# isl-org/Open3D-PointNet2-Semantic3D

Hardware: AMD Instinct MI355X
Metric: points/sec through SA+FP stack (B=16,N=8192) (higher is better)
Workload: dtype f32

## Files before the change

### open3d-pointnet2-semantic3d_amd/csrc/pn2_common.h

```cpp
#pragma once
#include <hip/hip_runtime.h>
#include <stdint.h>

#include "../../include/pn2_abi.h"
#include "pn2_device_set.h"

#define PN2_WAVE 64

#ifdef PN2_TUNING_HOOKS
#define PN2_TUNABLE(type, name, value) type name = value;
#else
#define PN2_TUNABLE(type, name, value) static constexpr type name = value;
#endif

#define PN2_RETURN_IF_LAUNCH_FAILED()                 \
    do {                                              \
        hipError_t e__ = hipGetLastError();           \
        if (e__ != hipSuccess) return (int)e__;       \
    } while (0)

constexpr int kPn2CuLdsBytes = 160 * 1024;
constexpr int kPn2DefaultDynLdsBytes = 64 * 1024;

template <auto Kern>
int pn2_allow_lds(int bytes) {
    static Pn2DeviceSet raised;
    int dev = -1;
    hipError_t e = hipGetDevice(&dev);
    if (e != hipSuccess) return (int)e;
    if (raised.done(dev)) return 0;
    e = hipFuncSetAttribute(reinterpret_cast<const void*>(Kern), hipFuncAttributeMaxDynamicSharedMemorySize, bytes);
    if (e != hipSuccess) return (int)e;
    raised.mark(dev);
    return 0;
}

constexpr int kPn2BnHead = 48;
constexpr int kPn2BnSlots = 64;
constexpr int kPn2BnTickets = 64;
#ifndef PN2_STREAM_MIN_ROWS
#define PN2_STREAM_MIN_ROWS 65536
#endif
#ifndef PN2_FOLD_DEPTH
#define PN2_FOLD_DEPTH 64
#endif
constexpr int kPn2FoldDepth = PN2_FOLD_DEPTH;
__host__ __device__ inline size_t pn2_bn_ws_doubles(int c, int nslots) { return kPn2BnHead + (size_t)(1 + nslots) * 2 * (size_t)c; }
inline bool pn2_bn_ws_fits(const void* ws, size_t bytes, int c) {
    return c > 0 && bytes >= sizeof(double) * pn2_bn_ws_doubles(c, kPn2BnSlots) && ((uintptr_t)ws % 8) == 0;
}

__device__ __forceinline__ void bn_scale_shift(float gamma, float beta, float mean, float invstd, float& sc, float& sh) {
    sc = gamma * invstd;
    sh = __builtin_fmaf(-mean, sc, beta);
}

struct Pn2BnFinish {
    int kind;
    int c, nslots;
    long long rows;
    double* ws;
    const float* gamma;
    const float* beta;
    const float* bias;
    const float* mean_in;
    const float* invstd_in;
    float eps, decay;
    float* running_mean;
    float* running_var;
    float* save_mean;
    float* save_invstd;
    float* scale;
    float* shift;
    float* coef;
    float* dgamma;
    float* dbeta;
};

__device__ __forceinline__ double pn2_load_device_scope(const double* p) {
    return __longlong_as_double((long long)__hip_atomic_load(reinterpret_cast<const unsigned long long*>(p), __ATOMIC_RELAXED,
                                                             __HIP_MEMORY_SCOPE_AGENT));
}

__device__ __forceinline__ void pn2_bn_finish(const Pn2BnFinish& f, unsigned nwg, unsigned wg) {
    if (f.kind == 0) return;
    __shared__ int s_last;
    asm volatile("s_waitcnt vmcnt(0)" ::: "memory");
    __syncthreads();
    if (threadIdx.x == 0) {
        unsigned* tick = reinterpret_cast<unsigned*>(f.ws);
        const unsigned g = wg % (unsigned)kPn2BnTickets;
        const unsigned ng = nwg < (unsigned)kPn2BnTickets ? nwg : (unsigned)kPn2BnTickets;
        const unsigned expect = nwg / kPn2BnTickets + (g < nwg % kPn2BnTickets ? 1u : 0u);
        int last = 0;
        if (__hip_atomic_fetch_add(tick + g, 1u, __ATOMIC_RELAXED, __HIP_MEMORY_SCOPE_AGENT) == expect - 1u)
            last = __hip_atomic_fetch_add(tick + kPn2BnTickets, 1u, __ATOMIC_RELAXED, __HIP_MEMORY_SCOPE_AGENT) == ng - 1u;
        s_last = last;
    }
    __syncthreads();
    if (!s_last) return;
    const int c = f.c;
    for (int col = threadIdx.x; col < 2 * c; col += blockDim.x) {
        double t = 0.0;
        const double* sl = f.ws + kPn2BnHead + (size_t)2 * c + col;
        int k = 0;
        for (; k + kPn2FoldDepth <= f.nslots; k += kPn2FoldDepth) {
            double v[kPn2FoldDepth];
#pragma unroll
            for (int u = 0; u < kPn2FoldDepth; ++u) v[u] = pn2_load_device_scope(sl + (size_t)2 * c * (k + u));
#pragma unroll
            for (int u = 0; u < kPn2FoldDepth; ++u) t += v[u];
        }
        for (; k < f.nslots; ++k) t += pn2_load_device_scope(sl + (size_t)2 * c * k);
        f.ws[kPn2BnHead + col] = t;
    }
    if (f.kind == 1) return;
    __threadfence_block();
    __syncthreads();
// ... 148 lines not shown
```

### open3d-pointnet2-semantic3d_amd/csrc/pn2_mlp_wide.hip

```cpp
#include "pn2_common.h"

namespace {

typedef float f32x4 __attribute__((ext_vector_type(4)));
typedef float f32x16 __attribute__((ext_vector_type(16)));

constexpr int kWideDepth = 4;

struct WideParams {
    int rows, cin, x_stride, nlayers, pool, relu_last;
    int w[3];
    const float* x;
    int n, m, c;
    const float* xyz;
    const float* new_xyz;
    const float* points;
    const int* idx;
    const float* dist;
    const float* points1;
    int c1, c2;
    const float* W[3];
    const float* bias[3];
    float* y;
    const float* zpre;
    int rowtab_off;
    int sa[2];
    int scratch_off;
    int scratch_alias;
};

enum { kWidePlain = 0, kWideGather = 1, kWideInterp = 2 };
template <int MODE>
__global__ void __launch_bounds__(256, 2)
mlp_wide_kernel(WideParams p) {
    constexpr bool GATHER = MODE == kWideGather;
    extern __shared__ __attribute__((aligned(16))) float smem[];
    const int tid = threadIdx.x;
    const int lane = tid & 63, half = lane >> 5, l31 = lane & 31;
    const int wave = __builtin_amdgcn_readfirstlane(tid >> 6);
    const int tile = blockIdx.x;
    const int row0 = tile * 32;
    const int buf_off[2] = {0, 32 * p.sa[0]};
    float* const buf0 = smem;

    struct LayerCfg { int N, wnt, ks_n, nq, ks, cb, g0, g1; const float* wcol; };
    auto make_cfg = [&](int l, int Kt) {
        LayerCfg c;
        c.N = p.w[l];
        c.wnt = c.N >> 7;
        c.ks_n = 4 / c.wnt;
        c.nq = wave % c.wnt;
        c.ks = wave / c.wnt;
        c.cb = c.nq * 128;
        const int ngroups = (Kt + 7) >> 3;
        c.g0 = (ngroups * c.ks) / c.ks_n;
        c.g1 = (ngroups * (c.ks + 1)) / c.ks_n;
        c.wcol = p.W[l] + c.cb + 4 * l31;
        return c;
    };
    f32x4 bq[kWideDepth][4];
    auto fetch_b = [&](const LayerCfg& c, int g, f32x4 (&b_)[4]) {
        const float* __restrict__ wp = c.wcol + (size_t)(8 * g + 4 * half) * c.N;
#pragma unroll
        for (int q = 0; q < 4; ++q) b_[q] = *reinterpret_cast<const f32x4*>(wp + (size_t)q * c.N);
    };
    auto prefetch_b = [&](const LayerCfg& c) {
#pragma unroll
        for (int u = 0; u < kWideDepth; ++u) fetch_b(c, c.g0 + u < c.g1 ? c.g0 + u : c.g1 - 1, bq[u]);
    };
    const LayerCfg first = make_cfg(0, p.cin);
    prefetch_b(first);

    const int K0 = (p.cin + 7) & ~7;
    auto stage4 = [&](int count4, int cv, int sa, auto src_of) {
        for (int base = 0; base < count4; base += 256 * 8) {
            f32x4 v[8];
#pragma unroll
            for (int u = 0; u < 8; ++u) {
                int e = base + u * 256 + tid;
                e = e < count4 ? e : count4 - 1;
                const int r = e / cv, j = e - r * cv;
                v[u] = *reinterpret_cast<const f32x4*>(src_of(r, j));
            }
#pragma unroll
            for (int u = 0; u < 8; ++u) {
                const int e = base + u * 256 + tid;
                if (e < count4) {
                    const int r = e / cv, j = e - r * cv;
                    *reinterpret_cast<f32x4*>(buf0 + r * sa + 4 * j) = v[u];
                }
            }
        }
    };
    if constexpr (GATHER) {
        const int c = p.c, cv = c >> 2;
        const int bi = tile / p.m;
        const float* __restrict__ pts = p.points + (size_t)bi * p.n * c;
        const int* __restrict__ idx = p.idx + (size_t)tile * 32;
        float* myrow = buf0 + (tid & 31) * p.sa[0];
        float dx = 0.f, dy = 0.f, dz = 0.f;
        if (tid < 32) {
            const float* __restrict__ q = p.xyz + ((size_t)bi * p.n + idx[tid]) * 3;
            const float* __restrict__ ctr = p.new_xyz + (size_t)tile * 3;
            dx = q[0] - ctr[0]; dy = q[1] - ctr[1]; dz = q[2] - ctr[2];
        }
        if (p.zpre) {
            if (tid < 32) {
                myrow[0] = dx; myrow[1] = dy; myrow[2] = dz;
                for (int k = 3; k < K0; ++k) myrow[k] = 0.f;
            }
        } else {
        stage4(32 * cv, cv, p.sa[0], [&](int r, int j) { return pts + (size_t)idx[r] * c + 4 * j; });
        if (tid < 32) {
            myrow[c] = dx; myrow[c + 1] = dy; myrow[c + 2] = dz;
            for (int k = c + 3; k < K0; ++k) myrow[k] = 0.f;
        }
        }
    } else if constexpr (MODE == kWideInterp) {
        const int c2 = p.c2, c1 = p.c1, cv2 = c2 >> 2, cv1 = c1 >> 2;
        const int bi = row0 / p.n;
        const float* __restrict__ p2 = p.points + (size_t)bi * p.m * c2;
        float* rowtab = smem + (p.zpre ? p.rowtab_off : buf_off[1]);
        if (tid < 32) {
            const size_t r = (size_t)row0 + tid;
            const float d1 = fmaxf(p.dist[r * 3 + 0], 1e-10f), d2 = fmaxf(p.dist[r * 3 + 1], 1e-10f);
            const float d3 = fmaxf(p.dist[r * 3 + 2], 1e-10f);
            const float r1 = 1.0f / d1, r2 = 1.0f / d2, r3 = 1.0f / d3;
            const float norm = (r1 + r2) + r3;
            *reinterpret_cast<f32x4*>(rowtab + tid * 8) = f32x4{r1 / norm, r2 / norm, r3 / norm, 0.f};
            *reinterpret_cast<f32x4*>(rowtab + tid * 8 + 4) =
                f32x4{__int_as_float(p.idx[r * 3 + 0]), __int_as_float(p.idx[r * 3 + 1]), __int_as_float(p.idx[r * 3 + 2]), 0.f};
        }
        __syncthreads();
        const int count4 = p.zpre ? 0 : 32 * cv2;
        for (int base = 0; base < count4; base += 256 * 4) {
            f32x4 v[4];
#pragma unroll
            for (int u = 0; u < 4; ++u) {
                int e = base + u * 256 + tid;
                e = e < count4 ? e : count4 - 1;
                const int r = e / cv2, j = e - r * cv2;
                const f32x4 wq = *reinterpret_cast<const f32x4*>(rowtab + r * 8);
                const f32x4 iq = *reinterpret_cast<const f32x4*>(rowtab + r * 8 + 4);
                const f32x4 x1 = *reinterpret_cast<const f32x4*>(p2 + (size_t)__float_as_int(iq[0]) * c2 + 4 * j);
                const f32x4 x2 = *reinterpret_cast<const f32x4*>(p2 + (size_t)__float_as_int(iq[1]) * c2 + 4 * j);
                const f32x4 x3 = *reinterpret_cast<const f32x4*>(p2 + (size_t)__float_as_int(iq[2]) * c2 + 4 * j);
                v[u] = (x1 * wq[0] + x2 * wq[1]) + x3 * wq[2];
            }
#pragma unroll
            for (int u = 0; u < 4; ++u) {
                const int e = base + u * 256 + tid;
                if (e < count4) {
                    const int r = e / cv2, j = e - r * cv2;
                    *reinterpret_cast<f32x4*>(buf0 + r * p.sa[0] + 4 * j) = v[u];
                }
            }
        }
        if (c1 > 0) {
            const float* __restrict__ p1 = p.points1 + (size_t)row0 * c1;
            for (int e = tid; e < 32 * cv1; e += 256) {
                const int r = e / cv1, j = e - r * cv1;
                *reinterpret_cast<f32x4*>(buf0 + r * p.sa[0] + (p.zpre ? 0 : c2) + 4 * j) = *reinterpret_cast<const f32x4*>(p1 + (size_t)r * c1 + 4 * j);
            }
        }
        if (K0 > p.cin) {
            const int padw = K0 - p.cin;
            for (int e = tid; e < 32 * padw; e += 256) buf0[(e / padw) * p.sa[0] + p.cin + e % padw] = 0.f;
        }
    } else {
        const float* __restrict__ x = p.x;
        if ((p.x_stride & 3) == 0 && (p.cin & 3) == 0 && (((uintptr_t)x) & 15) == 0) {
            const int cv = p.cin >> 2;
            stage4(32 * cv, cv, p.sa[0], [&](int r, int j) {
                const int gr = row0 + r < p.rows ? row0 + r : p.rows - 1;
                return x + (size_t)gr * p.x_stride + 4 * j;
            });
            if (row0 + 32 > p.rows) {
                __syncthreads();
                for (int e = tid; e < 32 * p.cin; e += 256) {
                    const int r = e / p.cin;
                    if (row0 + r >= p.rows) buf0[r * p.sa[0] + e - r * p.cin] = 0.f;
                }
            }
        } else {
// ... 50 lines not shown
            f32x4 aq[kWideDepth];
#pragma unroll
            for (int u = 0; u < kWideDepth; ++u) aq[u] = *reinterpret_cast<const f32x4*>(arow + 8 * (g0 + u < g1 ? g0 + u : last));
            int g = g0;
            for (; g + 2 * kWideDepth <= g1; g += kWideDepth) {
#pragma unroll
                for (int u = 0; u < kWideDepth; ++u) {
                    contract(aq[u], bq[u]);
                    __builtin_amdgcn_sched_barrier(0);
                    const int gn = g + kWideDepth + u;
                    aq[u] = *reinterpret_cast<const f32x4*>(arow + 8 * gn);
                    fetch_b(cur, gn, bq[u]);
                    __builtin_amdgcn_sched_barrier(0);
                }
            }
            const int rem = g1 - g - kWideDepth;
#pragma unroll
            for (int u = 0; u < kWideDepth; ++u) {
                if (g + u < g1) contract(aq[u], bq[u]);
                if (u < rem) {
                    aq[u] = *reinterpret_cast<const f32x4*>(arow + 8 * (g + kWideDepth + u));
                    fetch_b(cur, g + kWideDepth + u, bq[u]);
                }
            }
#pragma unroll
            for (int u = 0; u < kWideDepth - 1; ++u)
                if (u < rem) contract(aq[u], bq[u]);
        }
        const bool lastl = l == p.nlayers - 1;
        LayerCfg nxt = cur;
        if (!lastl) {
            nxt = make_cfg(l + 1, N);
            prefetch_b(nxt);
        }

        if (ks_n > 1) {
            const int sc_off = p.scratch_alias ? in_off : p.scratch_off;
            if (p.scratch_alias) __syncthreads();
            auto park = [&](int block) {
                float* dst = smem + sc_off + block * (64 * 64);
#pragma unroll
                for (int t = 0; t < 4; ++t)
#pragma unroll
                    for (int r = 0; r < 16; ++r) dst[(t * 16 + r) * 64 + lane] = acc[t][r];
            };
            auto add = [&](int block) {
                const float* src = smem + sc_off + block * (64 * 64);
#pragma unroll
                for (int t = 0; t < 4; ++t)
#pragma unroll
                    for (int r = 0; r < 16; ++r) acc[t][r] += src[(t * 16 + r) * 64 + lane];
            };
            if (ks_n == 4) {
                if (ks >= 2) park(ks - 2);
                __syncthreads();
                if (ks < 2) add(ks);
                __syncthreads();
                if (ks == 1) park(0);
                __syncthreads();
                if (ks == 0) add(0);
            } else {
                if (ks == 1) park(nq);
                __syncthreads();
                if (ks == 0) add(nq);
            }
        }
        if (ks == 0 && l == 0 && p.zpre) {
            if constexpr (MODE == kWideInterp) {
                const float* __restrict__ zb = p.zpre + (size_t)(row0 / p.n) * p.m * N + cb + 4 * l31;
                const float* rowtab = smem + p.rowtab_off;
#pragma unroll
                for (int r = 0; r < 16; ++r) {
                    const int row = (r & 3) + 8 * (r >> 2) + 4 * half;
                    const f32x4 wq = *reinterpret_cast<const f32x4*>(rowtab + row * 8);
                    const f32x4 iq = *reinterpret_cast<const f32x4*>(rowtab + row * 8 + 4);
                    const f32x4 z1 = *reinterpret_cast<const f32x4*>(zb + (size_t)__float_as_int(iq[0]) * N);
                    const f32x4 z2 = *reinterpret_cast<const f32x4*>(zb + (size_t)__float_as_int(iq[1]) * N);
                    const f32x4 z3 = *reinterpret_cast<const f32x4*>(zb + (size_t)__float_as_int(iq[2]) * N);
                    const f32x4 z = (z1 * wq[0] + z2 * wq[1]) + z3 * wq[2];
#pragma unroll
                    for (int t = 0; t < 4; ++t) acc[t][r] += z[t];
                }
            } else if constexpr (MODE == kWideGather) {
                const float* __restrict__ zb = p.zpre + (size_t)(tile / p.m) * p.n * N + cb + 4 * l31;
                const int* __restrict__ idx = p.idx + (size_t)tile * 32;
#pragma unroll
                for (int r = 0; r < 16; ++r) {
                    const int row = (r & 3) + 8 * (r >> 2) + 4 * half;
                    const f32x4 z = *reinterpret_cast<const f32x4*>(zb + (size_t)idx[row] * N);
#pragma unroll
                    for (int t = 0; t < 4; ++t) acc[t][r] += z[t];
                }
            }
        }
        if (ks == 0) {
            const f32x4 bv = *reinterpret_cast<const f32x4*>(p.bias[l] + cb + 4 * l31);
            const bool relu = !lastl || p.relu_last;
            if (!lastl) {
                float* __restrict__ out = smem + buf_off[(l + 1) & 1];
                const int so = p.sa[(l + 1) & 1];
#pragma unroll
                for (int r = 0; r < 16; ++r) {
                    const int row = (r & 3) + 8 * (r >> 2) + 4 * half;
                    f32x4 v = {acc[0][r] + bv[0], acc[1][r] + bv[1], acc[2][r] + bv[2], acc[3][r] + bv[3]};
                    v = {fmaxf(v[0], 0.f), fmaxf(v[1], 0.f), fmaxf(v[2], 0.f), fmaxf(v[3], 0.f)};
                    *reinterpret_cast<f32x4*>(out + row * so + cb + 4 * l31) = v;
                }
            } else if (p.pool == 32) {
                f32x4 v;
#pragma unroll
                for (int t = 0; t < 4; ++t) {
                    float mx = acc[t][0];
#pragma unroll
                    for (int r = 1; r < 16; ++r) mx = fmaxf(mx, acc[t][r]);
                    mx = fmaxf(mx, __shfl_xor(mx, 32));
                    mx += bv[t];
                    v[t] = relu ? fmaxf(mx, 0.f) : mx;
                }
                if (half == 0) *reinterpret_cast<f32x4*>(p.y + (size_t)tile * N + cb + 4 * l31) = v;
            } else {
#pragma unroll
                for (int r = 0; r < 16; ++r) {
                    const int row = row0 + (r & 3) + 8 * (r >> 2) + 4 * half;
                    f32x4 v = {acc[0][r] + bv[0], acc[1][r] + bv[1], acc[2][r] + bv[2], acc[3][r] + bv[3]};
                    if (relu) v = {fmaxf(v[0], 0.f), fmaxf(v[1], 0.f), fmaxf(v[2], 0.f), fmaxf(v[3], 0.f)};
                    if (row < p.rows) *reinterpret_cast<f32x4*>(p.y + (size_t)row * N + cb + 4 * l31) = v;
                }
            }
        }
        if (!lastl) __syncthreads();
        cur = nxt;
    }
}

template <int MODE>
int launch_mlp_wide_mode(const WideParams& p, size_t lds, hipStream_t st) {
    if (int e = pn2_allow_lds<mlp_wide_kernel<MODE>>(kPn2CuLdsBytes)) return e;
    mlp_wide_kernel<MODE><<<(p.rows + 31) / 32, 256, lds, st>>>(p);
    PN2_RETURN_IF_LAUNCH_FAILED();
    return PN2_OK;
}

int launch_mlp_wide(WideParams& p, int mode, hipStream_t st) {
    const int k0 = (p.cin + 7) & ~7;
    int ka = k0, kb = 0;
    if (p.nlayers >= 2) kb = p.w[0];
    if (p.nlayers >= 3 && p.w[1] > ka) ka = p.w[1];
    p.sa[0] = ka + 4;
    p.sa[1] = kb + 4 > 8 ? kb + 4 : 8;
    bool sliced = false, alias_ok = true;
    int kin = k0;
    for (int l = 0; l < p.nlayers; ++l) {
        if (p.w[l] < 512) {
            sliced = true;
            if ((size_t)32 * p.sa[l & 1] < (size_t)2 * 64 * 64) alias_ok = false;
        }
        kin = p.w[l];
    }
    (void)kin;
    p.scratch_off = 32 * (p.sa[0] + p.sa[1]);
    p.scratch_alias = sliced && alias_ok;
    p.rowtab_off = p.scratch_off + (sliced && !alias_ok ? 2 * 64 * 64 : 0);
    const size_t lds = sizeof(float) * ((size_t)p.rowtab_off + (p.zpre && mode == kWideInterp ? 32 * 8 : 0));
    if (lds > kPn2CuLdsBytes) return PN2_EUNSUP;
    if (mode == kWideGather) return launch_mlp_wide_mode<kWideGather>(p, lds, st);
    if (mode == kWideInterp) return launch_mlp_wide_mode<kWideInterp>(p, lds, st);
    return launch_mlp_wide_mode<kWidePlain>(p, lds, st);
}

int check_layers(int nlayers, const int* widths, const float* const* w, const float* const* bias) {
    if (nlayers < 1 || nlayers > 3) return PN2_EUNSUP;
    if (!widths || !w || !bias) return PN2_ENULL;
    for (int l = 0; l < nlayers; ++l) {
        if (widths[l] != 128 && widths[l] != 256 && widths[l] != 512) return PN2_EUNSUP;
        if (!w[l] || !bias[l]) return PN2_ENULL;
        if ((((uintptr_t)w[l]) | ((uintptr_t)bias[l])) & 15) return PN2_EUNSUP;
    }
    return PN2_OK;
}

}

extern "C" int pn2_mlp_wide(int rows, int cin, int x_stride, const float* x, int nlayers, const int* widths,
                            const float* const* w, const float* const* bias, int relu_last, int pool, float* y, void* stream) {
    if (rows <= 0 || cin <= 0 || x_stride < cin) return PN2_EINVAL;
    if (!x || !y) return PN2_ENULL;
    int rc = check_layers(nlayers, widths, w, bias);
    if (rc != PN2_OK) return rc;
    if (pool != 0 && pool != 32) return PN2_EUNSUP;
    if (pool == 32 && rows % 32 != 0) return PN2_EINVAL;
    if (((uintptr_t)y) & 15) return PN2_EUNSUP;
    if ((long long)rows + 64 > 0x7fffffffLL) return PN2_ERANGE;
    WideParams p = {};
    p.rows = rows; p.cin = cin; p.x_stride = x_stride; p.nlayers = nlayers; p.pool = pool; p.relu_last = relu_last;
    p.x = x; p.y = y;
    for (int l = 0; l < nlayers; ++l) { p.w[l] = widths[l]; p.W[l] = w[l]; p.bias[l] = bias[l]; }
    return launch_mlp_wide(p, kWidePlain, static_cast<hipStream_t>(stream));
}

extern "C" int pn2_sa_mlp_wide(int b, int n, int m, int nsample, int c, const float* xyz, const float* new_xyz,
                               const float* points, const int* idx, int nlayers, const int* widths, const float* const* w,
                               const float* const* bias, int pool, float* y, void* stream) {
    if (b <= 0 || n <= 0 || m <= 0 || c <= 0) return PN2_EINVAL;
    if (!xyz || !new_xyz || !points || !idx || !y) return PN2_ENULL;
    if (nsample != 32 || c % 4 != 0 || (((uintptr_t)points | (uintptr_t)y) & 15)) return PN2_EUNSUP;
    int rc = check_layers(nlayers, widths, w, bias);
    if (rc != PN2_OK) return rc;
    if ((long long)b * m * 32 + 64 > 0x7fffffffLL) return PN2_ERANGE;
    WideParams p = {};
    p.rows = b * m * 32; p.cin = 3 + c; p.x_stride = 0; p.nlayers = nlayers; p.pool = pool ? 32 : 0; p.relu_last = 1;
    p.n = n; p.m = m; p.c = c; p.xyz = xyz; p.new_xyz = new_xyz; p.points = points; p.idx = idx; p.y = y;
    for (int l = 0; l < nlayers; ++l) { p.w[l] = widths[l]; p.W[l] = w[l]; p.bias[l] = bias[l]; }
    return launch_mlp_wide(p, kWideGather, static_cast<hipStream_t>(stream));
}

extern "C" int pn2_fp_mlp_wide(int b, int n, int m, int c1, int c2, const float* dist, const int* idx, const float* points1,
                               const float* points2, int nlayers, const int* widths, const float* const* w,
                               const float* const* bias, float* y, void* stream) {
    if (b <= 0 || n <= 0 || m < 3 || c2 <= 0 || c1 < 0) return PN2_EINVAL;
    if (!dist || !idx || !points2 || !y || (c1 > 0 && !points1)) return PN2_ENULL;
    if (n % 32 != 0 || c2 % 4 != 0 || c1 % 4 != 0 || (((uintptr_t)points2 | (uintptr_t)points1 | (uintptr_t)y) & 15)) return PN2_EUNSUP;
    int rc = check_layers(nlayers, widths, w, bias);
    if (rc != PN2_OK) return rc;
    if ((long long)b * n + 64 > 0x7fffffffLL) return PN2_ERANGE;
    WideParams p = {};
    p.rows = b * n; p.cin = c2 + c1; p.nlayers = nlayers; p.pool = 0; p.relu_last = 1;
    p.n = n; p.m = m; p.c1 = c1; p.c2 = c2; p.dist = dist; p.idx = idx; p.points = points2; p.points1 = points1; p.y = y;
    for (int l = 0; l < nlayers; ++l) { p.w[l] = widths[l]; p.W[l] = w[l]; p.bias[l] = bias[l]; }
    return launch_mlp_wide(p, kWideInterp, static_cast<hipStream_t>(stream));
}

extern "C" int pn2_fp_mlp_wide_pre(int b, int n, int m, int c1, const float* dist, const int* idx, const float* points1,
                                   const float* z, int nlayers, const int* widths, const float* const* w,
                                   const float* const* bias, float* y, void* stream) {
    if (b <= 0 || n <= 0 || m < 3 || c1 <= 0) return PN2_EINVAL;
    if (!dist || !idx || !z || !y || !points1) return PN2_ENULL;
    if (n % 32 != 0 || c1 % 4 != 0 || (((uintptr_t)z | (uintptr_t)points1 | (uintptr_t)y) & 15)) return PN2_EUNSUP;
    int rc = check_layers(nlayers, widths, w, bias);
    if (rc != PN2_OK) return rc;
    if ((long long)b * n + 64 > 0x7fffffffLL) return PN2_ERANGE;
    WideParams p = {};
    p.rows = b * n; p.cin = c1; p.nlayers = nlayers; p.pool = 0; p.relu_last = 1;
    p.n = n; p.m = m; p.c1 = c1; p.c2 = 0; p.dist = dist; p.idx = idx; p.points = nullptr; p.points1 = points1; p.y = y; p.zpre = z;
    for (int l = 0; l < nlayers; ++l) { p.w[l] = widths[l]; p.W[l] = w[l]; p.bias[l] = bias[l]; }
    return launch_mlp_wide(p, kWideInterp, static_cast<hipStream_t>(stream));
}

// ... 16 lines not shown
```

### open3d-pointnet2-semantic3d_amd/csrc/pn2_sa_fused.hip

```cpp
#include "pn2_common.h"
#include <atomic>
#include <type_traits>
#include <utility>

namespace {

typedef float f32x4 __attribute__((ext_vector_type(4)));
typedef float f32x16 __attribute__((ext_vector_type(16)));

struct SaFusedParams {
    int n, m, c, groups;
    int kshift;
    int rows;
    int w[3];
    const float* xyz;
    const float* new_xyz;
    const float* points;
    const int* idx;
    const float* dist;
    const float* points1;
    int c1;
    int ldx, ldp, ld1;
    const float* W[3];
    const float* bias[3];
// ... 918 lines not shown
    const size_t bytes = floats * sizeof(float) + 64;
    if (bytes > 150 * 1024) return PN2_EUNSUP;
    const int need4 = (p.groups + 3) / 4;
    if constexpr (L == 1) {
        if (g_chain_nw == 16 && p.groups >= 4096) {
            constexpr auto kern = sa_fused_kernel<L, NT1, NT2, NT3, VEC8, DENSE, POOL, 16, INTERP, PREZ>;
            if (int e = pn2_allow_lds<kern>(kPn2CuLdsBytes)) return e;
            kern<<<g_chain_grid, 1024, bytes, st>>>(p);
            PN2_RETURN_IF_LAUNCH_FAILED();
            return PN2_OK;
        }
    }
    if constexpr (L == 3 && INTERP && PREZ && DENSE && !POOL && NT1 == 4) {
        const bool want_pipe = p.schedule < 0 ? g_chain_pipe != 0 : p.schedule == 1;
        if (p.schedule == 1 && p.c1 > 2 * kPipeSkipSteps) return PN2_EUNSUP;
        if (want_pipe && p.c1 <= 2 * kPipeSkipSteps && (p.groups >= 2048 || p.schedule == 1)) {
            const bool ns2 = p.c1 <= 4;
            auto kern = ns2 ? fp_chain_pipe_kernel<NT2, NT3, 2> : fp_chain_pipe_kernel<NT2, NT3, 4>;
            if (int e = ns2 ? pn2_allow_lds<fp_chain_pipe_kernel<NT2, NT3, 2>>(kPn2CuLdsBytes)
                            : pn2_allow_lds<fp_chain_pipe_kernel<NT2, NT3, 4>>(kPn2CuLdsBytes))
                return e;
            const size_t pbytes = ((size_t)(ns2 ? 2 : 4) * 2 * W1 + W1 + (size_t)W1 * W2 + W2 + (size_t)W2 * W3 + W3) * sizeof(float);
            int grid = g_chain_grid;
            if (grid > need4) grid = need4;
            kern<<<grid, 256, pbytes, st>>>(p);
            PN2_RETURN_IF_LAUNCH_FAILED();
            return PN2_OK;
        }
    }
    if constexpr (L == 3 && INTERP && PREZ) {
#ifdef PN2_FP4_NW12
        constexpr bool nw12 = true;
#else
        const bool nw12 = g_chain_nw == 12;
#endif
        if (nw12 && bytes > 78 * 1024 && p.groups >= 2048) {
            constexpr auto kern = sa_fused_kernel<L, NT1, NT2, NT3, VEC8, DENSE, POOL, 12, INTERP, PREZ>;
            if (int e = pn2_allow_lds<kern>(kPn2CuLdsBytes)) return e;
            int grid = g_chain_grid;
            const int need12 = (p.groups + 11) / 12;
            if (grid > need12) grid = need12;
            kern<<<grid, 768, bytes, st>>>(p);
            PN2_RETURN_IF_LAUNCH_FAILED();
            return PN2_OK;
        }
    }
    if (bytes > 78 * 1024 && p.groups >= 2048 && g_chain_nw != 4) {
        int e = 0;
        auto kern = chain_kernel<L, NT1, NT2, NT3, VEC8, DENSE, POOL, 8, INTERP, PREZ>(pack, e);
        if (e) return e;
        int grid = g_chain_grid;
        const int need8 = (p.groups + 7) / 8;
        if (grid > need8) grid = need8;
        p.blk = pack_block(p.groups, grid);
        kern<<<grid, 512, bytes + (pack ? kPackLdsBytes : 0), st>>>(p);
    } else {
        int e = 0;
        auto kern = chain_kernel<L, NT1, NT2, NT3, VEC8, DENSE, POOL, 4, INTERP, PREZ>(pack, e);
        if (e) return e;
        int grid = bytes > 78 * 1024 ? g_chain_grid : g_chain_grid * 2;
        if (grid > need4) grid = need4;
        p.blk = pack_block(p.groups, grid);
        kern<<<grid, 256, bytes + (pack ? kPackLdsBytes : 0), st>>>(p);
    }
    PN2_RETURN_IF_LAUNCH_FAILED();
    return PN2_OK;
}

}

#ifdef PN2_TUNING_HOOKS
extern "C" int pn2_debug_set_chain_stats(long long* dev_ptr) { g_chain_stats = dev_ptr; return 0; }
extern "C" int pn2_debug_set_chain_trace(long long* dev_ptr) { g_chain_trace = dev_ptr; return 0; }
extern "C" int pn2_debug_set_fused(int what, int value) {
    if (what == 6) { g_chain_grid = value; return 0; }
    if (what == 7) { g_chain_nw = value; return 0; }
    if (what == 13) { g_chain_prio = value; return 0; }
    if (what == 14) { g_chain_pipe = value; return 0; }
    if (what == 16) { g_chain_tag = value; return 0; }
    return PN2_EINVAL;
}
#endif

extern "C" int pn2_set_sa_row_packing(int on) {
    g_sa_row_packing.store(on != 0, std::memory_order_relaxed);
    return PN2_OK;
}

static int sa_fused_impl(int b, int n, int m, int nsample, int c, const float* xyz,
                         const float* new_xyz, const float* points, const int* idx,
                         int nlayers, const int* widths, const float* const* w,
                         const float* const* bias, float* out, bool pool, void* stream, int ld_xyz, int ld_points);

extern "C" int pn2_sa_mlp_max_fused(int b, int n, int m, int nsample, int c, const float* xyz,
                                    const float* new_xyz, const float* points, const int* idx,
                                    int nlayers, const int* widths, const float* const* w,
                                    const float* const* bias, float* out, void* stream) {
    return sa_fused_impl(b, n, m, nsample, c, xyz, new_xyz, points, idx, nlayers, widths, w, bias, out, true, stream, 3, c);
}

extern "C" int pn2_sa_mlp_max_fused_ld(int b, int n, int m, int nsample, int c, const float* xyz, int ld_xyz,
                                       const float* new_xyz, const float* points, int ld_points, const int* idx,
                                       int nlayers, const int* widths, const float* const* w,
                                       const float* const* bias, float* out, void* stream) {
    return sa_fused_impl(b, n, m, nsample, c, xyz, new_xyz, points, idx, nlayers, widths, w, bias, out, true, stream, ld_xyz,
                         c > 0 ? ld_points : 0);
}

extern "C" int pn2_sa_mlp_rows_fused(int b, int n, int m, int nsample, int c, const float* xyz,
                                     const float* new_xyz, const float* points, const int* idx,
                                     int nlayers, const int* widths, const float* const* w,
                                     const float* const* bias, float* out, void* stream) {
    return sa_fused_impl(b, n, m, nsample, c, xyz, new_xyz, points, idx, nlayers, widths, w, bias, out, false, stream, 3, c);
}

static int sa_fused_impl(int b, int n, int m, int nsample, int c, const float* xyz,
                         const float* new_xyz, const float* points, const int* idx,
                         int nlayers, const int* widths, const float* const* w,
                         const float* const* bias, float* out, bool pool, void* stream, int ld_xyz, int ld_points) {
    if (b <= 0 || n <= 0 || m <= 0 || nsample <= 0 || c < 0 || nlayers <= 0) return PN2_EINVAL;
    if (!xyz || !new_xyz || !idx || !widths || !w || !bias || !out || (c > 0 && !points)) return PN2_ENULL;
    if (nlayers > 3) return PN2_EUNSUP;
    int kshift = 0;
    while ((1 << kshift) < nsample) ++kshift;
    if ((1 << kshift) != nsample || kshift < 4 || kshift > 8) return PN2_EUNSUP;
    if (kshift != 5 && !pool) return PN2_EUNSUP;
    if (kshift == 4 && (((long long)b * m) & 1)) return PN2_EUNSUP;
    if ((long long)b * m * nsample > 0x7fffffffLL - 64) return PN2_ERANGE;
    SaFusedParams p{};
    p.schedule = -1;
    p.n = n; p.m = m; p.c = c; p.kshift = kshift;
    p.groups = (int)(((long long)b * m * nsample) / 32); p.rows = p.groups * 32;
    p.xyz = xyz; p.new_xyz = new_xyz; p.points = points; p.idx = idx; p.out = out;
    int nt[3] = {0, 0, 0};
    for (int l = 0; l < nlayers; ++l) {
        if (widths[l] <= 0 || widths[l] % 32 != 0 || widths[l] > 128) return PN2_EUNSUP;
        if (!w[l] || !bias[l]) return PN2_ENULL;
        if ((uintptr_t)w[l] % 16 != 0) return PN2_EUNSUP;
        p.w[l] = widths[l]; p.W[l] = w[l]; p.bias[l] = bias[l];
        nt[l] = widths[l] / 32;
    }
    const bool vec8 = c > 0 && (c % 8 == 0) && ((uintptr_t)points % 16 == 0);
    if (ld_xyz < 3 || (c > 0 && ld_points < c)) return PN2_EINVAL;
    if (vec8 && ld_points != c) return PN2_EUNSUP;
    p.ldx = ld_xyz; p.ldp = ld_points;
    hipStream_t st = static_cast<hipStream_t>(stream);
    if (kshift > 5) {
        hipError_t e = hipMemsetAsync(out, 0, sizeof(float) * (size_t)b * m * widths[nlayers - 1], st);
        if (e != hipSuccess) return (int)e;
    }
    const int key = nlayers * 1000 + nt[0] * 100 + nt[1] * 10 + nt[2];
    if (!pool) {
        if (key == 2440) return vec8 ? launch_chain<2, 4, 4, 1, true, false, false>(p, st)
                                     : launch_chain<2, 4, 4, 1, false, false, false>(p, st);
        if (key == 1400) return vec8 ? launch_chain<1, 4, 1, 1, true, false, false>(p, st)
                                     : launch_chain<1, 4, 1, 1, false, false, false>(p, st);
        return PN2_EUNSUP;
    }
#define PN2_SA_CASE(L_, A_, B_, C_)                                                     \
    case (L_ * 1000 + A_ * 100 + B_ * 10 + C_):                                         \
        return vec8 ? launch_chain<L_, A_, (B_ ? B_ : 1), (C_ ? C_ : 1), true, false, true>(p, st) \
                    : launch_chain<L_, A_, (B_ ? B_ : 1), (C_ ? C_ : 1), false, false, true>(p, st);
    switch (key) {
        PN2_SA_CASE(3, 1, 1, 2)
        PN2_SA_CASE(3, 2, 2, 4)
        PN2_SA_CASE(3, 2, 3, 4)
// ... 162 lines not shown
```

### open3d-pointnet2-semantic3d_amd/util/pointnet_util.py

```python

import torch

from . import tf_util
from .._lib import float_array, int_array, launch, lib, ptr, ptr_table, require_cuda, rows_in_place, u64_array
from ..tf_ops import tf_grouping
from ..tf_ops.tf_grouping import query_ball_point_multi, group_point, knn_point, query_ball_point
from ..tf_ops.tf_interpolate import three_interpolate, three_nn
from ..tf_ops.tf_sampling import (farthest_point_sample, farthest_point_sample_and_gather, farthest_point_sample_with_ties,
                                  gather_point, tag_fps_output)


def sample_and_group(npoint, radius, nsample, xyz, points, knn=False, use_xyz=True, geometry=None):
    plan = None
    if geometry is not None:
        new_xyz, idx = geometry[0], geometry[1]
        plan = geometry[2] if len(geometry) > 2 else None
    else:
        fps_idx, fps_tie, _ = farthest_point_sample_with_ties(npoint, xyz)
        new_xyz = tag_fps_output(gather_point(xyz, fps_idx), fps_tie)
        if knn:
            _, idx = knn_point(nsample, xyz, new_xyz)
        else:
            idx, pts_cnt = query_ball_point(radius, nsample, xyz, new_xyz)
    if USE_FUSED_TRAIN_FRONT and points is not None and use_xyz and points.dtype == torch.float32:
# ... 211 lines not shown
    _, new_xyz = farthest_point_sample_and_gather(npoint, xyz)
    idx, _ = query_ball_point(radius, nsample, xyz, new_xyz)
    return new_xyz, idx


USE_COARSE_GEOMETRY = True
COARSE_MAX_N, COARSE_MAX_LEVELS, COARSE_MAX_NN_M = 1024, 4, 256


def coarse_geometry_fits(n0, npoints, want_nn=True):
    if not USE_COARSE_GEOMETRY or not (0 < n0 <= COARSE_MAX_N) or not (0 < len(npoints) <= COARSE_MAX_LEVELS):
        return False
    n = n0
    for m in npoints:
        if not (0 < m <= n) or (want_nn and not (3 <= m <= COARSE_MAX_NN_M)):
            return False
        n = m
    return True


def coarse_geometry(xyz0, npoints, radii, nsamples, want_nn=True, fps_arith_mode=None, bq_arith_mode=None):
    from .. import config
    from ..tf_ops.tf_sampling import fps_tie_record
    require_cuda(xyz0)
    if xyz0.dim() != 3 or xyz0.shape[2] != 3 or xyz0.dtype != torch.float32:
        raise ValueError("coarse_geometry expects (batch_size,num_points,3) float32 xyz0")
    nlev = len(npoints)
    if not (len(radii) == len(nsamples) == nlev):
        raise ValueError("coarse_geometry expects one radius and one nsample per level")
    tie_in = fps_tie_record(xyz0, fps_arith_mode)
    xyz0 = xyz0.detach().contiguous()
    b, n0, _ = xyz0.shape
    dev = xyz0.device
    out, n = [], n0
    for m, ns in zip(npoints, nsamples):
        lv = {"new_xyz": torch.empty((b, m, 3), dtype=torch.float32, device=dev),
              "fps_idx": torch.empty((b, m), dtype=torch.int32, device=dev),
              "idx": torch.empty((b, m, ns), dtype=torch.int32, device=dev),
              "cnt": torch.empty((b, m), dtype=torch.int32, device=dev),
              "nn": (torch.empty((b, n, 3), dtype=torch.float32, device=dev),
                     torch.empty((b, n, 3), dtype=torch.int32, device=dev)) if want_nn else None}
        out.append(lv)
        n = m
    tie_out = torch.empty((b,), dtype=torch.int32, device=dev)
    launch("pn2_coarse_geometry", dev, b, n0, nlev, int_array(npoints), float_array(radii), int_array(nsamples), ptr(xyz0), ptr(tie_in),
           ptr_table([lv["fps_idx"] for lv in out]), ptr_table([lv["new_xyz"] for lv in out]), ptr_table([lv["idx"] for lv in out]),
           ptr_table([lv["cnt"] for lv in out]), ptr_table([lv["nn"][0] if want_nn else None for lv in out]),
           ptr_table([lv["nn"][1] if want_nn else None for lv in out]), ptr(tie_out), config.fps_mode(fps_arith_mode),
           config.bq_mode(bq_arith_mode))
    tag_fps_output(out[-1]["new_xyz"], tie_out, fps_arith_mode)
    return out


def sa_features_inference(xyz, new_xyz, points, idx, mlp, bn=True, bn_decay=None):
    nsample = idx.shape[2]
    new_points = None
    if USE_FUSED_SA:
        new_points = _sa_fused_inference(xyz, new_xyz, points, idx, mlp, bn, "conv%d")
    if new_points is None:
        xyz = xyz.contiguous()
        points = None if points is None else points.contiguous()
    if new_points is None and points is not None and points.dtype == torch.bfloat16:
        points = points.float()
        if USE_FUSED_SA:
            new_points = _sa_fused_inference(xyz, new_xyz, points, idx, mlp, bn, "conv%d")
    if new_points is None and USE_FUSED_SA and len(mlp) == 3 and mlp[0] == mlp[1] == 128 and mlp[2] % 32 == 0:
        h = _sa_fused_inference(xyz, new_xyz, points, idx, mlp[:2], bn, "conv%d", pool=False)
        if h is not None:
            h = tf_util.conv2d(h, mlp[2], [1, 1], padding="VALID", stride=[1, 1], bn=bn, is_training=False,
                               scope="conv2", bn_decay=bn_decay, pool=nsample)
            new_points = h.squeeze(2)
    if (new_points is None and USE_MLP_WIDE and USE_FUSED_SA and nsample == 32 and points is not None
            and points.dtype == torch.float32 and points.shape[2] % 4 == 0 and 1 <= len(mlp) <= 3
            and all(w in (128, 256, 512) for w in mlp) and idx.shape[0] * idx.shape[1] * 32 >= WIDE_MIN_ROWS):
        folded, cprev = [], 3 + points.shape[2]
        for i, cout in enumerate(mlp):
            with tf_util.variable_scope("conv%d" % i):
                if i == 0:
                    folded.append(tf_util.folded_dense(cprev, cout, bn, (1, 1, cprev, cout), pad_to=32,
                                                       pad_in=-(-cprev // 8) * 8, rotate_rows=cprev - 3))
                else:
                    folded.append(tf_util.folded_dense(cprev, cout, bn, (1, 1, cprev, cout), pad_to=32))
            cprev = cout
        if USE_HOISTED_SA:
            new_points = tf_util.hip_sa_mlp_wide_pre(xyz, new_xyz, points, idx, [f[0] for f in folded], [f[1] for f in folded])
        if new_points is None:
            new_points = tf_util.hip_sa_mlp_wide(xyz, new_xyz, points, idx, [f[0] for f in folded], [f[1] for f in folded])
    if new_points is None:
        h = _sa_group_concat(xyz, new_xyz, points, idx)
        pool_ok = nsample == 16 or nsample % 32 == 0
        for i, cout in enumerate(mlp):
            last = i == len(mlp) - 1
            h = tf_util.conv2d(h, cout, [1, 1], padding="VALID", stride=[1, 1], bn=bn, is_training=False,
                               scope="conv%d" % i, bn_decay=bn_decay, pool=nsample if (last and pool_ok) else 0)
        if not pool_ok:
            h = h.amax(dim=2, keepdim=True)
        new_points = h.squeeze(2)
    return new_points


_POOL_MODES = {"max": 0, "avg": 1, "weighted_avg": 2, "max_and_avg": 3}


class _GroupPool(torch.autograd.Function):
    @staticmethod
    def forward(ctx, x, gxyz, mode):
        b, m, k, c = x.shape
        x = x.contiguous()
        gxyz = gxyz.contiguous() if gxyz is not None else None
        out = torch.empty((b, m, 1, 2 * c if mode == 3 else c), dtype=torch.float32, device=x.device)
        launch("pn2_group_pool", x, b * m, k, c, mode, ptr(x), ptr(gxyz), ptr(out))
        ctx.save_for_backward(x, gxyz if gxyz is not None else x.new_empty(0))
        ctx.mode = mode
        return out

    @staticmethod
    def backward(ctx, dout):
        x, gxyz = ctx.saved_tensors
        b, m, k, c = x.shape
        dx = torch.empty_like(x)
        launch("pn2_group_pool_grad", x, b * m, k, c, ctx.mode, ptr(x), ptr(gxyz if gxyz.numel() else None), ptr(dout.contiguous()),
               ptr(dx))
        return dx, None, None


def group_pool(new_points, grouped_xyz, pooling):
    mode = _POOL_MODES[pooling]
    require_cuda(new_points)
    if new_points.dtype != torch.float32:
        raise TypeError("pooling expects float32 features")
    tf_util.assert_not_deferred(new_points, "a pooling")
    return _GroupPool.apply(new_points, grouped_xyz if mode == 2 else None, mode)


def pointnet_sa_module(xyz, points, npoint, radius, nsample, mlp, mlp2, group_all, is_training, bn_decay, scope,
                       bn=True, pooling="max", knn=False, use_xyz=True, use_nchw=False, geometry=None):
    require_cuda(xyz, points)
    with tf_util.variable_scope(scope):
        if not is_training and not group_all and not knn and use_xyz and pooling == "max":
            if geometry is not None and geometry[1] is None:
                new_xyz = geometry[0]
                if len(geometry) > 2 and geometry[2] is not None:
                    idx, _ = tf_grouping.query_ball_point_binned(radius, nsample, xyz, new_xyz, geometry[2])
                else:
                    idx, _ = query_ball_point(radius, nsample, xyz, new_xyz)
            else:
                new_xyz, idx = geometry[:2] if geometry is not None else sa_geometry(xyz, npoint, radius, nsample)
            new_points = sa_features_inference(xyz, new_xyz, points, idx, mlp, bn, bn_decay)
            new_points = new_points.unsqueeze(2)
        else:
            if geometry is not None and geometry[1] is None:
                raise ValueError("geometry=(new_xyz, None) (samples drawn ahead, ball query here) is the inference fast path's "
                                 "hand-over: pass the idx too for training / group_all / knn / non-max pooling")
            hoist = (bool(is_training) and tf_util.USE_HOISTED_TRAIN and not group_all and not knn and use_xyz and bn
                     and pooling == "max" and points is not None and points.dtype == torch.float32 and points.shape[2] >= 16
                     and len(mlp) > 0 and mlp[0] % 4 == 0 and nsample <= 1024 and geometry is not None and len(geometry) > 2
                     and _plan_usable(geometry[2], mlp[0]))
            first = 0
            defer = lambda i, rows: (bool(is_training) and bn and i + 1 < len(mlp)
                                     and tf_util.can_defer_bn(rows, mlp[i], mlp[i + 1]))
            small_first = (bool(is_training) and tf_util.USE_SA_FIRST_LAYER_FUSED and tf_util.USE_BN_FINISH_IN_PRODUCER
                           and not hoist and not group_all and not knn and use_xyz and bn and pooling == "max"
                           and points is not None and points.dtype == torch.float32 and points.shape[2] <= 5
                           and not points.requires_grad and len(mlp) > 0 and mlp[0] % 4 == 0 and mlp[0] <= 1024
                           and nsample <= 1024)
            if small_first:
# ... 268 lines not shown
```

Measured before the change: 370.8 million.

## Pack sparse SA ball-query groups into shared wide-MLP tiles

Adds a packing variant of the gathered wide-MLP kernel. Each block classifies a chunk of 256 ball-query groups by how many distinct leading neighbours they have (8, 16 or 32, using the padding that repeats the first index). It then packs two or four small groups into one 32-row tile and max-pools per slot. Blocks beyond the packed tile count exit early. This saves MLP work on duplicated padded rows, at the cost of extra index scanning, ballots and syncs per block, and it only runs when the row-packing flag is set.

```diff
diff --git a/open3d-pointnet2-semantic3d_amd/csrc/pn2_common.h b/open3d-pointnet2-semantic3d_amd/csrc/pn2_common.h
--- a/open3d-pointnet2-semantic3d_amd/csrc/pn2_common.h
+++ b/open3d-pointnet2-semantic3d_amd/csrc/pn2_common.h
@@ -34,6 +34,8 @@
     raised.mark(dev);
     return 0;
 }
+
+__attribute__((visibility("hidden"))) bool pn2_sa_row_packing_enabled();
 
 constexpr int kPn2BnHead = 48;
 constexpr int kPn2BnSlots = 64;
diff --git a/open3d-pointnet2-semantic3d_amd/csrc/pn2_mlp_wide.hip b/open3d-pointnet2-semantic3d_amd/csrc/pn2_mlp_wide.hip
--- a/open3d-pointnet2-semantic3d_amd/csrc/pn2_mlp_wide.hip
+++ b/open3d-pointnet2-semantic3d_amd/csrc/pn2_mlp_wide.hip
@@ -30,10 +30,13 @@
 };
 
 enum { kWidePlain = 0, kWideGather = 1, kWideInterp = 2 };
-template <int MODE>
+constexpr int kPackChunk = 256;
+constexpr int kPackRows = 0, kPackGroups = 32, kPackMeta = 36, kPackCounts = 40, kPackLdsInts = 64;
+template <int MODE, bool PACK = false>
 __global__ void __launch_bounds__(256, 2)
 mlp_wide_kernel(WideParams p) {
     constexpr bool GATHER = MODE == kWideGather;
+    static_assert(!PACK || GATHER, "PACK: the pooled gather mode only");
     extern __shared__ __attribute__((aligned(16))) float smem[];
     const int tid = threadIdx.x;
     const int lane = tid & 63, half = lane >> 5, l31 = lane & 31;
@@ -69,7 +72,72 @@
         for (int u = 0; u < kWideDepth; ++u) fetch_b(c, c.g0 + u < c.g1 ? c.g0 + u : c.g1 - 1, bq[u]);
     };
     const LayerCfg first = make_cfg(0, p.cin);
-    prefetch_b(first);
+    int* const pk = reinterpret_cast<int*>(smem + p.rowtab_off);
+    (void)pk;
+    if constexpr (PACK) {
+        const int groups = p.rows >> 5;
+        const int cbase = (tile / kPackChunk) * kPackChunk, mytile = tile - cbase;
+        const int cnt = min(kPackChunk, groups - cbase);
+        int cls = 0;
+        if (tid < cnt) {
+            const int4* __restrict__ ip = reinterpret_cast<const int4*>(p.idx + (size_t)(cbase + tid) * 32);
+            int4 v[8];
+#pragma unroll
+            for (int u = 0; u < 8; ++u) v[u] = ip[u];
+            const int head = v[0].x;
+            int live = 1;
+#pragma unroll
+            for (int u = 0; u < 8; ++u) {
+                if (v[u].x != head) live = 4 * u + 1;
+                if (v[u].y != head) live = 4 * u + 2;
+                if (v[u].z != head) live = 4 * u + 3;
+                if (v[u].w != head) live = 4 * u + 4;
+            }
+            cls = live <= 8 ? 8 : (live <= 16 ? 16 : 32);
+        }
+        const unsigned long long m32 = __ballot(cls == 32), m16 = __ballot(cls == 16), m8 = __ballot(cls == 8);
+        if (lane == 0) {
+            pk[kPackCounts + 3 * wave + 0] = __popcll(m32);
+            pk[kPackCounts + 3 * wave + 1] = __popcll(m16);
+            pk[kPackCounts + 3 * wave + 2] = __popcll(m8);
+        }
+        __syncthreads();
+        int n32 = 0, n16 = 0, n8 = 0, b32 = 0, b16 = 0, b8 = 0;
+#pragma unroll
+        for (int w = 0; w < 4; ++w) {
+            const int c32 = pk[kPackCounts + 3 * w], c16 = pk[kPackCounts + 3 * w + 1], c8 = pk[kPackCounts + 3 * w + 2];
+            n32 += c32; n16 += c16; n8 += c8;
+            if (w < wave) { b32 += c32; b16 += c16; b8 += c8; }
+        }
+        n32 = __builtin_amdgcn_readfirstlane(n32); n16 = __builtin_amdgcn_readfirstlane(n16); n8 = __builtin_amdgcn_readfirstlane(n8);
+        const int promote = ((n16 & 1) && (n8 & 3) == 1) ? 1 : 0;
+        const int k16 = n16 + promote, k8 = n8 - promote, t16 = (k16 + 1) >> 1;
+        const int ntiles = n32 + t16 + ((k8 + 3) >> 2);
+        if (mytile >= ntiles) return;
+        prefetch_b(first);
+        if (cls != 0) {
+            const unsigned long long below = (1ull << lane) - 1ull;
+            int t, slot;
+            if (cls == 32) { t = b32 + __popcll(m32 & below); slot = 0; }
+            else {
+                int c = cls, r = cls == 16 ? b16 + __popcll(m16 & below) : b8 + __popcll(m8 & below);
+                if (promote && c == 8 && r == n8 - 1) { c = 16; r = n16; }
+                if (c == 16) { t = n32 + (r >> 1); slot = r & 1; }
+                else { t = n32 + t16 + (r >> 2); slot = r & 3; }
+            }
+            if (t == mytile) pk[kPackGroups + slot] = cbase + tid;
+        }
+        if (tid == 0) {
+            int sshift, nvalid;
+            if (mytile < n32) { sshift = 5; nvalid = 1; }
+            else if (mytile < n32 + t16) { sshift = 4; nvalid = min(2, k16 - 2 * (mytile - n32)); }
+            else { sshift = 3; nvalid = min(4, k8 - 4 * (mytile - n32 - t16)); }
+            pk[kPackMeta] = sshift; pk[kPackMeta + 1] = nvalid;
+        }
+        __syncthreads();
+    } else {
+        prefetch_b(first);
+    }
 
     const int K0 = (p.cin + 7) & ~7;
     auto stage4 = [&](int count4, int cv, int sa, auto src_of) {
@@ -94,12 +162,24 @@
     };
     if constexpr (GATHER) {
         const int c = p.c, cv = c >> 2;
-        const int bi = tile / p.m;
+        const int bi = PACK ? 0 : tile / p.m;
         const float* __restrict__ pts = p.points + (size_t)bi * p.n * c;
-        const int* __restrict__ idx = p.idx + (size_t)tile * 32;
+        const int* __restrict__ idx = PACK ? pk + kPackRows : p.idx + (size_t)tile * 32;
         float* myrow = buf0 + (tid & 31) * p.sa[0];
         float dx = 0.f, dy = 0.f, dz = 0.f;
-        if (tid < 32) {
+        if constexpr (PACK) {
+            if (tid < 32) {
+                const int sshift = pk[kPackMeta], nvalid = pk[kPackMeta + 1];
+                const int q = tid >> sshift;
+                const int g = pk[kPackGroups + (q < nvalid ? q : 0)];
+                const int src = (g / p.m) * p.n + p.idx[(size_t)g * 32 + (tid & ((1 << sshift) - 1))];
+                pk[kPackRows + tid] = src;
+                const float* __restrict__ q3 = p.xyz + (size_t)src * 3;
+                const float* __restrict__ ctr = p.new_xyz + (size_t)g * 3;
+                dx = q3[0] - ctr[0]; dy = q3[1] - ctr[1]; dz = q3[2] - ctr[2];
+            }
+            __syncthreads();
+        } else if (tid < 32) {
             const float* __restrict__ q = p.xyz + ((size_t)bi * p.n + idx[tid]) * 3;
             const float* __restrict__ ctr = p.new_xyz + (size_t)tile * 3;
             dx = q[0] - ctr[0]; dy = q[1] - ctr[1]; dz = q[2] - ctr[2];
@@ -316,8 +396,8 @@
                     for (int t = 0; t < 4; ++t) acc[t][r] += z[t];
                 }
             } else if constexpr (MODE == kWideGather) {
-                const float* __restrict__ zb = p.zpre + (size_t)(tile / p.m) * p.n * N + cb + 4 * l31;
-                const int* __restrict__ idx = p.idx + (size_t)tile * 32;
+                const float* __restrict__ zb = p.zpre + (PACK ? (size_t)0 : (size_t)(tile / p.m) * p.n * N) + cb + 4 * l31;
+                const int* __restrict__ idx = PACK ? pk + kPackRows : p.idx + (size_t)tile * 32;
 #pragma unroll
                 for (int r = 0; r < 16; ++r) {
                     const int row = (r & 3) + 8 * (r >> 2) + 4 * half;
@@ -340,6 +420,37 @@
                     v = {fmaxf(v[0], 0.f), fmaxf(v[1], 0.f), fmaxf(v[2], 0.f), fmaxf(v[3], 0.f)};
                     *reinterpret_cast<f32x4*>(out + row * so + cb + 4 * l31) = v;
                 }
+            } else if constexpr (PACK) {
+                const int sshift = __builtin_amdgcn_readfirstlane(pk[kPackMeta]);
+                const int nvalid = __builtin_amdgcn_readfirstlane(pk[kPackMeta + 1]);
+                f32x4 qm[4];
+#pragma unroll
+                for (int q = 0; q < 4; ++q)
+#pragma unroll
+                    for (int t = 0; t < 4; ++t) {
+                        const float mx = fmaxf(fmaxf(acc[t][4 * q], acc[t][4 * q + 1]), fmaxf(acc[t][4 * q + 2], acc[t][4 * q + 3]));
+                        qm[q][t] = fmaxf(mx, __shfl_xor(mx, 32));
+                    }
+                auto store = [&](int slot, const f32x4& mx) {
+                    if (half == 0 && slot < nvalid) {
+                        f32x4 v = mx + bv;
+                        if (relu) v = {fmaxf(v[0], 0.f), fmaxf(v[1], 0.f), fmaxf(v[2], 0.f), fmaxf(v[3], 0.f)};
+                        const int g = pk[kPackGroups + slot];
+                        *reinterpret_cast<f32x4*>(p.y + (size_t)g * N + cb + 4 * l31) = v;
+                    }
+                };
+                auto vmax = [](const f32x4& a, const f32x4& b) {
+                    return f32x4{fmaxf(a[0], b[0]), fmaxf(a[1], b[1]), fmaxf(a[2], b[2]), fmaxf(a[3], b[3])};
+                };
+                if (sshift == 3) {
+#pragma unroll
+                    for (int q = 0; q < 4; ++q) store(q, qm[q]);
+                } else if (sshift == 4) {
+                    store(0, vmax(qm[0], qm[1]));
+                    store(1, vmax(qm[2], qm[3]));
+                } else {
+                    store(0, vmax(vmax(qm[0], qm[1]), vmax(qm[2], qm[3])));
+                }
             } else if (p.pool == 32) {
                 f32x4 v;
 #pragma unroll
@@ -367,10 +478,10 @@
     }
 }
 
-template <int MODE>
+template <int MODE, bool PACK = false>
 int launch_mlp_wide_mode(const WideParams& p, size_t lds, hipStream_t st) {
-    if (int e = pn2_allow_lds<mlp_wide_kernel<MODE>>(kPn2CuLdsBytes)) return e;
-    mlp_wide_kernel<MODE><<<(p.rows + 31) / 32, 256, lds, st>>>(p);
+    if (int e = pn2_allow_lds<mlp_wide_kernel<MODE, PACK>>(kPn2CuLdsBytes)) return e;
+    mlp_wide_kernel<MODE, PACK><<<(p.rows + 31) / 32, 256, lds, st>>>(p);
     PN2_RETURN_IF_LAUNCH_FAILED();
     return PN2_OK;
 }
@@ -395,8 +506,11 @@
     p.scratch_off = 32 * (p.sa[0] + p.sa[1]);
     p.scratch_alias = sliced && alias_ok;
     p.rowtab_off = p.scratch_off + (sliced && !alias_ok ? 2 * 64 * 64 : 0);
-    const size_t lds = sizeof(float) * ((size_t)p.rowtab_off + (p.zpre && mode == kWideInterp ? 32 * 8 : 0));
+    const bool pack = mode == kWideGather && p.pool == 32 && pn2_sa_row_packing_enabled() && (((uintptr_t)p.idx) & 15) == 0 &&
+                      (long long)(p.rows / 32 / p.m) * p.n <= 0x7fffffffLL;
+    const size_t lds = sizeof(float) * ((size_t)p.rowtab_off + (p.zpre && mode == kWideInterp ? 32 * 8 : 0) + (pack ? kPackLdsInts : 0));
     if (lds > kPn2CuLdsBytes) return PN2_EUNSUP;
+    if (pack) return launch_mlp_wide_mode<kWideGather, true>(p, lds, st);
     if (mode == kWideGather) return launch_mlp_wide_mode<kWideGather>(p, lds, st);
     if (mode == kWideInterp) return launch_mlp_wide_mode<kWideInterp>(p, lds, st);
     return launch_mlp_wide_mode<kWidePlain>(p, lds, st);
diff --git a/open3d-pointnet2-semantic3d_amd/csrc/pn2_sa_fused.hip b/open3d-pointnet2-semantic3d_amd/csrc/pn2_sa_fused.hip
--- a/open3d-pointnet2-semantic3d_amd/csrc/pn2_sa_fused.hip
+++ b/open3d-pointnet2-semantic3d_amd/csrc/pn2_sa_fused.hip
@@ -1024,6 +1024,8 @@
 }
 #endif
 
+bool pn2_sa_row_packing_enabled() { return g_sa_row_packing.load(std::memory_order_relaxed) != 0; }
+
 extern "C" int pn2_set_sa_row_packing(int on) {
     g_sa_row_packing.store(on != 0, std::memory_order_relaxed);
     return PN2_OK;
diff --git a/open3d-pointnet2-semantic3d_amd/util/pointnet_util.py b/open3d-pointnet2-semantic3d_amd/util/pointnet_util.py
--- a/open3d-pointnet2-semantic3d_amd/util/pointnet_util.py
+++ b/open3d-pointnet2-semantic3d_amd/util/pointnet_util.py
@@ -317,6 +317,7 @@
                 else:
                     folded.append(tf_util.folded_dense(cprev, cout, bn, (1, 1, cprev, cout), pad_to=32))
             cprev = cout
+        _sync_sa_row_packing(xyz)
         if USE_HOISTED_SA:
             new_points = tf_util.hip_sa_mlp_wide_pre(xyz, new_xyz, points, idx, [f[0] for f in folded], [f[1] for f in folded])
         if new_points is None:
```

After: 383.0 million, median of 6. 1.03x the previous value.
